# JJKK1313/DiTreeOnlinePlanner

Hardware: AMD Instinct MI355X
Metric: candidate tree-expansions/sec (carmaze, H=32) (higher is better)
Workload: dtype f16x3; 1 GPU; cfgs/carmaze.yaml + fm_policy flow sampler (K=1), batch=1024 candidates per GPU, H=32 (4 chunks x 8 steps), boxes.csv 20x20, 1024-node tree snapshot, seeded random weights; batch_per_gpu=1024, global_batch=1024, edge_length=32, action_horizon=8, pred_horizon=64, flow_steps=1, tree_nodes=1024, parallelism=candidates sharded x1

## Files before the change

ditreeonlineplanner_amd/csrc/conv_tiles.hip:

```cpp
#include <type_traits>

#include "denoise_device.h"

static thread_local bool g_dn_dry_run = false;
void denoise_set_dry_run(bool on) { g_dn_dry_run = on; }
bool denoise_dry_run() { return g_dn_dry_run; }

template <int PREC>
__device__ __forceinline__ void gemm_epilogue(const ConvGemmParams& p, f32x16_t (&acc)[2][4], char* smem, int tm, int tn,
                                              int tid, int lane, int r5, int h, int wm, int wn,
                                              long long out_extra_bytes = 0) {

  constexpr int ET = PREC == 2 ? 1 : 0;
  float satm = 0.0f;
  const int c_l = wn * 128 + 4 * r5;
  const int n0 = tn * 256 + c_l;
  const bool n_ok = n0 < p.N;
  float bias4[4] = {0.f, 0.f, 0.f, 0.f};
  if (p.bias != nullptr && n_ok) {
    f32x4_t t = *(const f32x4_t*)(p.bias + n0);
#pragma unroll
    for (int j = 0; j < 4; ++j) bias4[j] = t[j];
  }
#pragma unroll
// ... 1185 lines not shown
#pragma unroll
  for (int q = 0; q < 4; ++q) issue_w(v_lo, 1, q);
  rdA(0, v_lo, 0, 0);
  rdB(0, v_lo, 0, 1, 0);
#ifdef HALO16_STAMP
  const unsigned long long xs1 = __builtin_amdgcn_s_memrealtime();
#endif

  using IT1 = std::integral_constant<int, NP == 6 ? 3 : 2>;
  for (int v = v_lo; v < nv - 2; ++v) {
    step(I0{}, Tt{}, Tt{}, Tt{}, I3{}, v);
    step(I1{}, Tt{}, Tt{}, Tt{}, IT1{}, v);
    step(I2{}, Tt{}, Tt{}, Tt{}, I0{}, v);
  }
#ifdef X3_PHASE_STAMP
  if (blockIdx.x == 100 && lane == 0 && nv == 64) {
#pragma unroll
    for (int k = 0; k < 24; ++k) g_x3_phase[w][k] = pst[k];
    g_x3_phase[w][24] = (unsigned)nv;
  }
#endif
  {
    const int v = nv - 2;
    step(I0{}, Tt{}, Tt{}, Tt{}, I0{}, v);
    step(I1{}, Tt{}, Tt{}, Tt{}, I0{}, v);
    step(I2{}, Tt{}, Tt{}, Ff{}, I0{}, v);
  }
  {
    const int v = nv - 1;
    step(I0{}, Tt{}, Tt{}, Ff{}, I0{}, v);
    step(I1{}, Tt{}, Ff{}, Ff{}, I0{}, v);
    step(I2{}, Ff{}, Ff{}, Ff{}, I0{}, v);
  }
  __builtin_amdgcn_s_setprio(0);
  __syncthreads();
#ifdef HALO16_STAMP
  const unsigned long long xs2 = __builtin_amdgcn_s_memrealtime();
#endif
  if constexpr (SPLITK) {
    const int ntiles = ntm * ntn;
    float* mine = p.sk_ws + ((size_t)blockIdx.y * ntiles + tile) * 65536;
#pragma unroll
    for (int mb = 0; mb < 4; ++mb)
#pragma unroll
      for (int j = 0; j < 8; ++j) *(f32x4_t*)(mine + ((mb * 8 + j) * 512 + tid) * 4) = acc[mb][j];
    __threadfence();
    __syncthreads();
    int* s_last = (int*)smem;
    if (tid == 0) *s_last = atomicAdd(p.sk_cnt + tile, 1) == p.splitk - 1;
    __syncthreads();
    const bool last = *s_last != 0;
    __syncthreads();
    if (!last) return;
    __threadfence();
#pragma unroll
    for (int mb = 0; mb < 4; ++mb)
#pragma unroll
      for (int j = 0; j < 8; ++j) acc[mb][j] = f32x4_t{0.f, 0.f, 0.f, 0.f};
    for (int sp = 0; sp < p.splitk; ++sp) {
      const float* sl = p.sk_ws + ((size_t)sp * ntiles + tile) * 65536;
#pragma unroll
      for (int mb = 0; mb < 4; ++mb)
#pragma unroll
        for (int j = 0; j < 8; ++j) acc[mb][j] += *(const f32x4_t*)(sl + ((mb * 8 + j) * 512 + tid) * 4);
    }
    if (tid == 0) p.sk_cnt[tile] = 0;
  }
  gemm_epilogue16<ET, true, SHORT>(p, acc, smem, tm, tn, tid, lane, r4, h4, wm, wn);
#ifdef HALO16_STAMP
  __syncthreads();
  if (tid == 0) {
    const unsigned long long xs3 = __builtin_amdgcn_s_memrealtime();
    const unsigned int k = atomicAdd(&g_x3_count, 1u);
    if (k < X3_STAMP_MAX) {
      g_x3_stamp[k][0] = xs0; g_x3_stamp[k][1] = xs1; g_x3_stamp[k][2] = xs2; g_x3_stamp[k][3] = xs3;
      g_x3_stamp[k][4] = ((unsigned long long)nv << 32) | blockIdx.x;
      g_x3_stamp[k][5] = ((unsigned long long)__builtin_amdgcn_s_getreg((31 << 11) | 20) << 32) |
                         (unsigned int)__builtin_amdgcn_s_getreg((31 << 11) | 4);
    }
  }
#endif
}

template <int ET, bool SPLIT>
__global__ void __launch_bounds__(256) conv2d_small_kernel(ConvGemmParams p) {
  extern __shared__ __attribute__((aligned(16))) char smem[];
  constexpr int STAGE = 16384;
  constexpr int CK = SPLIT ? 32 : 64;
  const int tid = threadIdx.x, lane = tid & 63;
  const int w = __builtin_amdgcn_readfirstlane(tid >> 6);
  const int r5 = lane & 31, h = lane >> 5;
  const int wm = w >> 1, wn = w & 1;
  const int ntn = p.N >> 6;
  const int tm = blockIdx.x / ntn, tn = blockIdx.x - tm * ntn;
  const int kpt = p.Cin / CK;
  const long long K = (long long)p.taps * p.Cin;
  int k0 = 0, nk = p.taps * kpt;
  long long out_extra = 0;
  if (p.splitk > 1) {
    const int per = (nk + p.splitk - 1) / p.splitk;
    k0 = blockIdx.y * per;
    nk = min(nk - k0, per);
    out_extra = (long long)blockIdx.y * p.slab_stride;
  }

  const char* a_base[2];
  int ih0[2], iw0[2];
  const char* w_src[2];
  int slot_b[2];
  long long plane_a[2];
#pragma unroll
  for (int q = 0; q < 2; ++q) {
    const int r = (2 * w + q) * 8 + (lane >> 3);
    const int slot = (lane & 7) ^ ((r >> 1) & 7);
    slot_b[q] = SPLIT ? (slot & 3) * 16 : slot * 16;
    plane_a[q] = (SPLIT && (slot & 4)) ? p.a_plane : 0;
    const long long plane_w = (SPLIT && (slot & 4)) ? p.w_plane : 0;
    int m = tm * 64 + r;
    m = m < p.M ? m : p.M - 1;
    const int b = m / p.c2_OHW, rem = m - b * p.c2_OHW;
    const int oh = rem / p.c2_OW, ow = rem - oh * p.c2_OW;
    a_base[q] = (const char*)p.A + (long long)b * p.c2_H * p.c2_W * p.Cin * 2;
    ih0[q] = oh * p.c2_stride - p.c2_pad;
    iw0[q] = ow * p.c2_stride - p.c2_pad;
    w_src[q] = (const char*)p.W + ((long long)(tn * 64 + r) * K) * 2 + slot_b[q] + plane_w;
  }
  auto issue = [&](int kl) {
    const int k = k0 + kl;
    const int tap = k / kpt, kin = k - tap * kpt;
    const int kh = p.c2_kh[tap], kw = p.c2_kw[tap];
    char* st = smem + (kl % 3) * STAGE;
#pragma unroll
    for (int q = 0; q < 2; ++q) {
      const int ih = ih0[q] + kh, iw = iw0[q] + kw;
      const bool ok = ih >= 0 && ih < p.c2_H && iw >= 0 && iw < p.c2_W;
      const char* src = ok ? a_base[q] + ((long long)(ih * p.c2_W + iw) * p.Cin + kin * CK) * 2 + plane_a[q] : (const char*)p.zero;
      __builtin_amdgcn_global_load_lds((const GLOBAL_AS void*)(src + slot_b[q]), (LDS_AS void*)(st + (2 * w + q) * 1024), 16, 0, 0);
    }
#pragma unroll
    for (int q = 0; q < 2; ++q)
      __builtin_amdgcn_global_load_lds((const GLOBAL_AS void*)(w_src[q] + (long long)k * (CK * 2)),
                                       (LDS_AS void*)(st + 8192 + (2 * w + q) * 1024), 16, 0, 0);
  };

  f32x16_t acc;
#pragma unroll
  for (int i = 0; i < 16; ++i) acc[i] = 0.0f;
  const int a_row = wm * 32 + r5, b_row = wn * 32 + r5;
  const int a_off = a_row * 128, b_off = 8192 + b_row * 128;
  const int sa = (a_row >> 1) & 7, sb = (b_row >> 1) & 7;

  issue(0);
  if (nk > 1) issue(1);
  for (int k = 0; k < nk; ++k) {
    if (k + 1 < nk) asm volatile("s_waitcnt vmcnt(4)" ::: "memory");
    else asm volatile("s_waitcnt vmcnt(0)" ::: "memory");
    __builtin_amdgcn_s_barrier();
    if (k + 2 < nk) issue(k + 2);
    const char* st = smem + (k % 3) * STAGE;
    if constexpr (SPLIT) {
      short8_t af[4], bf[4];
#pragma unroll
      for (int ks = 0; ks < 4; ++ks) {
        af[ks] = *(const short8_t*)(st + a_off + ((((ks << 1) | h) ^ sa) << 4));
        bf[ks] = *(const short8_t*)(st + b_off + ((((ks << 1) | h) ^ sb) << 4));
      }
#pragma unroll
      for (int kk = 0; kk < 2; ++kk) acc = mfma32<ET>(af[kk], bf[kk + 2], acc);
#pragma unroll
      for (int kk = 0; kk < 2; ++kk) acc = mfma32<ET>(af[kk], bf[kk], acc);
#pragma unroll
      for (int kk = 0; kk < 2; ++kk) acc = mfma32<ET>(af[kk + 2], bf[kk], acc);
    } else {
#pragma unroll
      for (int ks = 0; ks < 4; ++ks) {
        const short8_t af = *(const short8_t*)(st + a_off + ((((ks << 1) | h) ^ sa) << 4));
        const short8_t bf = *(const short8_t*)(st + b_off + ((((ks << 1) | h) ^ sb) << 4));
        acc = mfma32<ET>(af, bf, acc);
      }
    }
    asm volatile("s_waitcnt lgkmcnt(0)" ::: "memory");
  }

  const int n = tn * 64 + wn * 32 + r5;
  float bias = (p.bias != nullptr && k0 == 0) ? p.bias[n] : 0.0f;
#pragma unroll
  for (int i = 0; i < 16; ++i) {
    const int m = tm * 64 + wm * 32 + (i & 3) + 8 * (i >> 2) + 4 * h;
    if (m < p.M) ((float*)p.Out)[out_extra + (long long)m * p.ldc + p.out_coff + n] = (ET == 1 ? acc[i] * p.w_scale : acc[i]) + bias;
  }
}

template <int ET, bool SPLIT, bool SHORT = false>
__global__ void __launch_bounds__(512, 2) gemm16_kernel(ConvGemmParams p) {
  extern __shared__ __attribute__((aligned(16))) char smem[];
  constexpr int BUF = 32768, W_BASE = 2 * BUF;
  const int tid = threadIdx.x, lane = tid & 63;
  const int w = __builtin_amdgcn_readfirstlane(tid >> 6);
  const int r4 = lane & 15, h4 = lane >> 4;
  const int wm = w >> 1, wn = w & 1;
  const int ntn = p.N >> 8, ntm = p.M >> 8;
  const int tile = xcd_remap_strips(blockIdx.x, ntm, ntn, p.xcd_strips);
  const int tm = tile / ntn, tn = tile - tm * ntn;
  constexpr int KB = SPLIT ? 64 : 128;
  const int nc = SPLIT ? (p.Cin >> 5) : (p.Cin >> 6), nk = p.taps * nc;
  const unsigned a_plane = (unsigned)p.a_plane, w_plane = (unsigned)p.w_plane;
  const long long K = (long long)p.taps * p.Cin;

  long long a_tile0;
  {
    const int m0 = tm * 256;
    const int b0 = m0 / p.L, l0 = m0 - b0 * p.L;
    a_tile0 = (((long long)b0 * p.in_Lp + (long long)l0 * p.in_stride + p.in_off) * p.lda) * 2;
  }
  const __amdgpu_buffer_rsrc_t a_rsrc =
      __builtin_amdgcn_make_buffer_rsrc((void*)((const char*)p.A + a_tile0), 0, 0x7fffffff, 0x00020000);
  const __amdgpu_buffer_rsrc_t w_rsrc =
      __builtin_amdgcn_make_buffer_rsrc((void*)((const char*)p.W + ((long long)tn * 256) * K * 2), 0, 0x7fffffff, 0x00020000);
  unsigned pae, pao, pbe, pbo;
  int aq[4], wq[4];
  {
    const int lr = lane >> 3;
    const int slot0 = (lane & 7) ^ (lr >> 1), slot1 = slot0 ^ 4;
    const int lrb = lr / p.L, lro = lrb * p.in_Lp + (lr - lrb * p.L) * p.in_stride;
    if constexpr (SPLIT) {
      pae = (unsigned)((lro * p.lda + (slot0 & 3) * 8) * 2) + ((slot0 & 4) ? a_plane : 0u);
      pao = (unsigned)((lro * p.lda + (slot1 & 3) * 8) * 2) + ((slot1 & 4) ? a_plane : 0u);
      pbe = (unsigned)(((long long)(8 * lr) * K + (slot0 & 3) * 8) * 2) + ((slot0 & 4) ? w_plane : 0u);
      pbo = (unsigned)(((long long)(8 * lr) * K + (slot1 & 3) * 8) * 2) + ((slot1 & 4) ? w_plane : 0u);
    } else {
      pae = (unsigned)((lro * p.lda + slot0 * 8) * 2);
      pao = (unsigned)((lro * p.lda + slot1 * 8) * 2);
      pbe = (unsigned)(((long long)(8 * lr) * K + slot0 * 8) * 2);
      pbo = (unsigned)(((long long)(8 * lr) * K + slot1 * 8) * 2);
    }
#pragma unroll
    for (int q = 0; q < 4; ++q) {
      const int r0 = (w * 4 + q) * 8;
      const int m = tm * 256 + r0;
      const int b = m / p.L, l = m - b * p.L;
      aq[q] = (int)((((long long)b * p.in_Lp + (long long)l * p.in_stride + p.in_off) * p.lda) * 2 - a_tile0);
      const int cu = (r0 & 128) + 8 * (r0 & 8) + ((r0 >> 4) & 7);
      wq[q] = (int)((long long)cu * K * 2);
    }
  }
  const int tap_bytes = p.lda * 2;
  auto src_off = [&](int k, int& ao, int& wo) {
    const int t = k / nc, c = k - t * nc;
    ao = t * tap_bytes + c * KB;
    wo = k * KB;
  };
  auto issue = [&](int kv) {
    int ao, wo;
    src_off(kv, ao, wo);
    char* ab = smem + (kv & 1) * BUF;
    char* wb = smem + W_BASE + (kv & 1) * BUF;
#pragma unroll
    for (int q = 0; q < 4; ++q)
      __builtin_amdgcn_raw_ptr_buffer_load_lds(a_rsrc, (LDS_AS void*)(ab + (w * 4 + q) * 1024), 16, (q & 1) ? pao : pae,
                                               aq[q] + ao, 0, 0);
#pragma unroll
    for (int q = 0; q < 4; ++q)
      __builtin_amdgcn_raw_ptr_buffer_load_lds(w_rsrc, (LDS_AS void*)(wb + (w * 4 + q) * 1024), 16, (q & 1) ? pbo : pbe,
                                               wq[q] + wo, 0, 0);
  };

// ... 78 lines not shown
      __builtin_amdgcn_sched_barrier(0);
      mm16(0, 1, 1);
      __builtin_amdgcn_sched_barrier(0);
    } else {
      rdB(1, k, 0, 1);
      mm16(0, 0, 0);
      __builtin_amdgcn_sched_group_barrier(0x100, 4, 0);
      __builtin_amdgcn_sched_group_barrier(0x008, 16, 0);
      __builtin_amdgcn_sched_barrier(0);
      rdA(1, k, 1);
      rdB(0, k, 1, 0);
      mm16(0, 1, 1);
      __builtin_amdgcn_sched_group_barrier(0x100, 8, 0);
      __builtin_amdgcn_sched_group_barrier(0x008, 16, 0);
      __builtin_amdgcn_sched_barrier(0);
      rdB(1, k, 1, 1);
      mm16(1, 0, 0);
      __builtin_amdgcn_sched_group_barrier(0x100, 4, 0);
      __builtin_amdgcn_sched_group_barrier(0x008, 16, 0);
      __builtin_amdgcn_sched_barrier(0);
    }
    int ao2 = 0, wo2 = 0;
    if constexpr (ISSUE) src_off(k + 2, ao2, wo2);
    if constexpr (HAS_NEXT) {
      asm volatile("s_waitcnt vmcnt(0) lgkmcnt(0)" ::: "memory");
      __builtin_amdgcn_s_barrier();
      rdA(0, k + 1, 0);
      rdB(0, k + 1, SPLIT ? 1 : 0, 0);
    }
#pragma unroll
    for (int mb = 0; mb < 4; ++mb)
#pragma unroll
      for (int jj = 0; jj < 4; ++jj) {
        mm(1, 1, 1, mb, (mb & 1) ? 3 - jj : jj);
        if constexpr (ISSUE) {
          const int m = mb * 4 + jj, i = (m & 1) ? -1 : (m >> 1);
          if (i >= 0 && i < 4)
            __builtin_amdgcn_raw_ptr_buffer_load_lds(a_rsrc, (LDS_AS void*)(smem + (k & 1) * BUF + (w * 4 + i) * 1024), 16,
                                                     (i & 1) ? pao : pae, aq[i] + ao2, 0, 0);
          else if (!SPLIT && i >= 4 && i < 8)
            __builtin_amdgcn_raw_ptr_buffer_load_lds(w_rsrc, (LDS_AS void*)(smem + W_BASE + (k & 1) * BUF + (w * 4 + i - 4) * 1024),
                                                     16, ((i - 4) & 1) ? pbo : pbe, wq[i - 4] + wo2, 0, 0);
        }
      }
    if constexpr (HAS_NEXT) __builtin_amdgcn_sched_group_barrier(0x100, 8, 1);
#pragma unroll
    for (int i = 0; i < 16; ++i) {
      __builtin_amdgcn_sched_group_barrier(0x008, 1, 1);
      if (ISSUE && !(i & 1) && (!SPLIT || i < 8)) __builtin_amdgcn_sched_group_barrier(0x020, 1, 1);
    }
    __builtin_amdgcn_sched_barrier(0);
  };
  using Tt = std::true_type;
  using Ff = std::false_type;

  issue(0);
  asm volatile("s_waitcnt vmcnt(0)" ::: "memory");
  __builtin_amdgcn_s_barrier();
  if (nk > 1) {
    if constexpr (SPLIT) {
      int ao, wo;
      src_off(1, ao, wo);
#pragma unroll
      for (int q = 0; q < 4; ++q)
        __builtin_amdgcn_raw_ptr_buffer_load_lds(a_rsrc, (LDS_AS void*)(smem + BUF + (w * 4 + q) * 1024), 16, (q & 1) ? pao : pae,
                                                 aq[q] + ao, 0, 0);
    } else {
      issue(1);
    }
  }
  rdA(0, 0, 0);
  rdB(0, 0, SPLIT ? 1 : 0, 0);
  for (int k = 0; k < nk - 2; ++k) step(Tt{}, Tt{}, k);
  if (nk >= 2) step(Tt{}, Ff{}, nk - 2);
  step(Ff{}, Ff{}, nk - 1);
  __syncthreads();
  gemm_epilogue16<ET, SPLIT, SHORT>(p, acc, smem, tm, tn, tid, lane, r4, h4, wm, wn);
}
enum { TILE_HALO, TILE_GEMM16, TILE_C2D_SMALL, TILE_GENERIC };
enum { TV_SPLIT = 1,
       TV_SHORT = 2,
       TV_SPLITK = 4,
       TV_NP6 = 8,
       TV_C2D = 16 };
struct TileVariant {
  void (*kernel)(ConvGemmParams);
  unsigned lds_bytes;
  unsigned block;
  int family, st;
  unsigned flags;
  int kind;
};
static const TileVariant k_tiles[] = {
    {conv3_halo16_kernel<0>, 147456, 512, TILE_HALO, ST_BF16, 0, 0},
    {conv3_halo16_kernel<1>, 147456, 512, TILE_HALO, ST_F16, 0, 0},
    {conv3_halo16x3_kernel<0>, 147456, 512, TILE_HALO, ST_BF16, TV_SPLIT, 0},
    {conv3_halo16x3_kernel<1>, 147456, 512, TILE_HALO, ST_F16, TV_SPLIT, 0},
    {conv3_halo16x3_kernel<0, true>, 147456, 512, TILE_HALO, ST_BF16, TV_SPLIT | TV_SHORT, 0},
    {conv3_halo16x3_kernel<1, true>, 147456, 512, TILE_HALO, ST_F16, TV_SPLIT | TV_SHORT, 0},
    {conv3_halo16x3_kernel<0, false, true>, 147456, 512, TILE_HALO, ST_BF16, TV_SPLIT | TV_SPLITK, 0},
    {conv3_halo16x3_kernel<1, false, true>, 147456, 512, TILE_HALO, ST_F16, TV_SPLIT | TV_SPLITK, 0},
    {conv3_halo16x3_kernel<0, true, true>, 147456, 512, TILE_HALO, ST_BF16, TV_SPLIT | TV_SHORT | TV_SPLITK, 0},
    {conv3_halo16x3_kernel<1, true, true>, 147456, 512, TILE_HALO, ST_F16, TV_SPLIT | TV_SHORT | TV_SPLITK, 0},
    {conv3_halo16x3_kernel<0, true, false, 6>, 163840, 512, TILE_HALO, ST_BF16, TV_SPLIT | TV_SHORT | TV_NP6, 0},
    {conv3_halo16x3_kernel<1, true, false, 6>, 163840, 512, TILE_HALO, ST_F16, TV_SPLIT | TV_SHORT | TV_NP6, 0},
    {gemm16_kernel<0, false>, 131072, 512, TILE_GEMM16, ST_BF16, 0, 1},
    {gemm16_kernel<1, false>, 131072, 512, TILE_GEMM16, ST_F16, 0, 1},
    {gemm16_kernel<0, true>, 131072, 512, TILE_GEMM16, ST_BF16, TV_SPLIT, 1},
    {gemm16_kernel<1, true>, 131072, 512, TILE_GEMM16, ST_F16, TV_SPLIT, 1},
    {gemm16_kernel<0, false, true>, 131072, 512, TILE_GEMM16, ST_BF16, TV_SHORT, 1},
    {gemm16_kernel<1, false, true>, 131072, 512, TILE_GEMM16, ST_F16, TV_SHORT, 1},
    {gemm16_kernel<0, true, true>, 131072, 512, TILE_GEMM16, ST_BF16, TV_SPLIT | TV_SHORT, 1},
    {gemm16_kernel<1, true, true>, 131072, 512, TILE_GEMM16, ST_F16, TV_SPLIT | TV_SHORT, 1},
    {conv2d_small_kernel<0, false>, 3 * 16384, 256, TILE_C2D_SMALL, ST_BF16, TV_C2D, 2},
    {conv2d_small_kernel<1, false>, 3 * 16384, 256, TILE_C2D_SMALL, ST_F16, TV_C2D, 2},
    {conv2d_small_kernel<0, true>, 3 * 16384, 256, TILE_C2D_SMALL, ST_BF16, TV_C2D | TV_SPLIT, 2},
    {conv2d_small_kernel<1, true>, 3 * 16384, 256, TILE_C2D_SMALL, ST_F16, TV_C2D | TV_SPLIT, 2},
    {conv_gemm_kernel<0, false>, 131072, 512, TILE_GENERIC, ST_BF16, 0, 1},
    {conv_gemm_kernel<1, false>, 131072, 512, TILE_GENERIC, ST_F32, 0, 1},
    {conv_gemm_kernel<2, false>, 131072, 512, TILE_GENERIC, ST_F16, 0, 1},
    {conv_gemm_kernel<0, true>, 131072, 512, TILE_GENERIC, ST_BF16, TV_C2D, 2},
    {conv_gemm_kernel<1, true>, 131072, 512, TILE_GENERIC, ST_F32, TV_C2D, 2},
    {conv_gemm_kernel<2, true>, 131072, 512, TILE_GENERIC, ST_F16, TV_C2D, 2},
};
static const TileVariant* find_tile(int family, int st, unsigned flags) {
  for (const TileVariant& v : k_tiles)
    if (v.family == family && v.st == st && v.flags == flags) return &v;
  return nullptr;
}

static const TileVariant* pick_tile(const ConvGemmParams& p, int fmt) {
  const int st = fmt_st(fmt);
  const bool split = fmt_split(fmt);
  const unsigned fsplit = split ? TV_SPLIT : 0;
  const bool tile16 = st != ST_F32 && !p.c2d && (p.M & 255) == 0 && (p.N & 255) == 0 && (p.Cin & 63) == 0;
  const bool l_ok = p.L >= 16 || (p.L == 8 && split) || (p.L == 4 && split && p.splitk <= 1);
  if (tile16 && p.taps == 3 && p.in_stride == 1 && p.in_Lp == p.L + 2 && (256 % p.L) == 0 && l_ok && p.Cin >= 192) {
    if (!split) return find_tile(TILE_HALO, st, 0);
    const unsigned fshort = p.L <= 8 ? TV_SHORT : 0;
    if (p.splitk > 1) return find_tile(TILE_HALO, st, TV_SPLIT | fshort | TV_SPLITK);
    return find_tile(TILE_HALO, st, TV_SPLIT | fshort | (p.L == 4 ? TV_NP6 : 0));
  }
  const bool short_l = p.L == 8 || p.L == 4;
  if (tile16 && (!p.out_f32 || p.mode == MODE_BIAS) && p.taps >= 1 && p.taps <= 3 && ((p.L & 15) == 0 || short_l) && p.M > 0 &&
      (p.mode == MODE_BIAS || (256 % p.L) == 0))
    return find_tile(TILE_GEMM16, st, fsplit | ((p.L & 15) != 0 ? TV_SHORT : 0));
  if (p.c2d && conv2d_small_eligible(fmt) && (p.N & 63) == 0 && (p.Cin & 63) == 0 && p.out_f32 && p.mode == MODE_BIAS)
    return find_tile(TILE_C2D_SMALL, st, TV_C2D | fsplit);
  if (split) return nullptr;
  return find_tile(TILE_GENERIC, st, p.c2d ? TV_C2D : 0);
}
bool conv2d_small_eligible(int fmt) { return fmt_st(fmt) != ST_F32; }
int conv_gemm_kind(const ConvGemmParams& p, int fmt) {
  const TileVariant* v = pick_tile(p, fmt);
  return v != nullptr ? v->kind : (p.c2d ? 2 : 1);
}
bool conv_gemm_supported(const ConvGemmParams& p, int fmt) { return pick_tile(p, fmt) != nullptr; }

static void ensure_lds_attrs() {
  static bool done[64] = {};
  int dev = 0;
  hipGetDevice(&dev);
  if (dev < 0 || dev >= 64 || done[dev]) return;
  done[dev] = true;
  for (const TileVariant& v : k_tiles)
    if (v.lds_bytes > 65536) hipFuncSetAttribute((const void*)v.kernel, hipFuncAttributeMaxDynamicSharedMemorySize, (int)v.lds_bytes);
}

void launch_conv_gemm(const ConvGemmParams& p, int fmt, hipStream_t s) {
  ensure_lds_attrs();
  const TileVariant* v = pick_tile(p, fmt);
  if (v != nullptr && (v->flags & TV_SPLITK) &&
      (p.sk_ws == nullptr || p.sk_cnt == nullptr || ((p.Cin >> 5) % p.splitk) != 0 || (p.Cin >> 5) / p.splitk < 2))
    throw std::runtime_error("conv_gemm: split-K of the halo kernel needs its workspace and splitk | Cin / 32, >= 2 chunks each");
  if ((v == nullptr || v->family == TILE_GENERIC) && p.mode >= MODE_GN_MISH && (p.L & 15) != 0)
    throw std::runtime_error("conv_gemm: a fused GroupNorm epilogue at L = 8 / 4 exists on the gemm16 tile only (whole 256-row tiles)");
  if (v == nullptr) throw std::runtime_error("conv_gemm: a split GEMM of this shape fits no tile (conv_gemm_supported is the contract)");
  dim3 grid(((p.M + 255) >> 8) * ((p.N + 255) >> 8));
  if (v->family == TILE_C2D_SMALL) grid.x = ((p.M + 63) >> 6) * (p.N >> 6);
  if (v->flags & (TV_SPLITK | TV_C2D)) grid.y = p.splitk > 1 ? p.splitk : 1;
  DN_LAUNCH(v->kernel, grid, dim3(v->block), v->lds_bytes, s, p);
}
```

ditreeonlineplanner_amd/csrc/denoise.h:

```cpp
#pragma once
#include <hip/hip_runtime.h>
#include <stdint.h>

enum { MODE_BIAS = 0, MODE_GN_MISH = 1, MODE_GN_MISH_FILM = 2, MODE_GN_MISH_RES = 3 };

enum { ST_BF16 = 0, ST_F32 = 1, ST_F16 = 2 };
static inline int fmt_make(int st, bool split) { return st | (split ? 4 : 0); }
static inline __host__ __device__ int fmt_st(int f) { return f & 3; }
static inline __host__ __device__ bool fmt_split(int f) { return (f & 4) != 0; }
static inline int fmt_es(int f) { return fmt_st(f) == ST_F32 ? 4 : 2; }

struct ConvGemmParams {
  const void* A;
  int lda;
  int in_Lp;
  int in_stride;
  int in_off;
  int taps, Cin;
  const void* W;
  void* Out;
  int ldc;
  int out_Lp, out_stride, out_off;
  int out_coff;
  int L;
  int M, N;
  const float* bias;
  int mode;
  const float* gamma;
  const float* beta;
  int group_ch;
  float eps;
  const float* film;
  int film_ld, film_off;
  const void* Res;
  int ldres, res_Lp, res_off;
  int out_f32;
  int xcd_strips;
  int c2d, c2_H, c2_W, c2_OW, c2_OHW, c2_stride, c2_pad;
  signed char c2_kh[12], c2_kw[12];
  const void* zero;
  long long a_plane, w_plane, out_plane, res_plane;
  float w_scale;
  int splitk;
  long long slab_stride;
  float* sk_ws;
  int* sk_cnt;
  int* sat;
};

void denoise_set_dry_run(bool on);
bool denoise_dry_run();
void launch_conv_gemm(const ConvGemmParams& p, int fmt, hipStream_t s);
bool conv2d_small_eligible(int fmt);
int conv_gemm_kind(const ConvGemmParams& p, int fmt);
bool conv_gemm_supported(const ConvGemmParams& p, int fmt);
void launch_prep_sample(const float* x, void* A0, int B, int P, int D, int fmt, long long plane, hipStream_t s, int* sat = nullptr);
void launch_time_embed(float t, const float* W1, const float* b1, const float* W2, const float* b2, float* out,
                       hipStream_t s);
void launch_prep_cond(const float* temb, const float* map_emb, int E, int E_ld, const float* cond, int G, void* out, int B,
                      int Kpad, int fmt, long long plane, hipStream_t s, int* sat = nullptr);
struct FlowStep {
  int mode;
  float dt;
  float sb, sa, c0, c1, sigma;
  const float* z;
  long long z_row;
  const int* z_idx;
  int z_row0;
};
void launch_final_proj_flow(const void* Y, int C, int Lp, long long plane, const float* W, const float* bias, int D, float* x,
                            FlowStep fs, const double* act_norm , double* actions, int B, int P, int fmt,
                            hipStream_t s);
struct TapList {
  int n;
  signed char kh[49], kw[49];
};
void launch_gn1d(void* x, int ld, int Lp, int row_off, int coff, int L, int C, const float* gamma, const float* beta, float eps,
                 int mode, const float* film, int film_ld, int film_off, const void* res, int ldres, int res_Lp, int res_off,
                 int B, int fmt, long long x_plane, long long res_plane, hipStream_t s, int* sat = nullptr);
void launch_encoder_stem(const float* lm, int n, const float* W, const float* gamma, const float* beta, void* out, int B, float eps,
                         int fmt, long long plane, hipStream_t s, int* sat = nullptr);
void launch_im2col2d(const void* in, bool src_f32, void* out, int B, int H, int W, int C, const TapList& taps, int stride,
                     int pad, int OH, int OW, int Kpad, int fmt, hipStream_t s);
void launch_gn2d(const float* in, int nslab, long long slab_stride, const float* gamma, const float* beta, const void* res,
                 int relu, void* out, int B, int HW, int C, float eps, int fmt, long long res_plane, long long out_plane,
                 hipStream_t s, int* sat = nullptr);
void launch_maxpool2d(const void* in, void* out, int B, int H, int W, int C, int OH, int OW, int fmt, hipStream_t s);
void launch_avgpool2d(const void* in, void* out, int B, int HW, int C, int fmt, long long in_plane, long long out_plane,
                      hipStream_t s);
void launch_unpack_act(const void* in, int ld, int coff, int Lp, int roff, float* out, int B, int L, int C, int fmt,
                       long long plane, hipStream_t s);

enum { ENC_RESNET = 0, ENC_IDENTITY = 1, ENC_MLP = 2, ENC_MAX = 3, ENC_GRID = 4, ENC_CNN = 5 };
struct SmallEncoderParams {
  int kind;
  const float* lm;
  float* out;
  int B, n, E, k;
  const float* w[4];
  const float* b[4];
};
const char* small_encoder_name(int kind);
int small_encoder_width(int kind, int n, int k);
void launch_small_encoder(const SmallEncoderParams& p, hipStream_t s);
```

ditreeonlineplanner_amd/csrc/denoise_host.hip:

```cpp
#include <algorithm>
#include <cmath>
#include <cstring>
#include <functional>
#include <map>
#include <sstream>
#include <thread>

#include "denoise.h"
#include "ditree_internal.h"

namespace {

struct HostParam {
  std::vector<int64_t> dims;
  const float* data = nullptr;
  int64_t n = 0;
};

struct Act {
  void* p = nullptr;
  int L = 0, C = 0;
  int ld = 0, coff = 0;
  bool padded = true;
  long long plane = 0;
// ... 599 lines not shown
    q.kind = enc_kind; q.n = lm; q.E = E; q.k = enc_k;
    auto transposed = [&](const std::string& name, int out_f, int in_f) {
      const HostParam& w = P_(name);
      if (w.dims.size() != 2 || w.dims[0] != out_f || w.dims[1] != in_f)
        throw std::runtime_error(name + " must be (" + std::to_string(out_f) + ", " + std::to_string(in_f) + ")");
      std::vector<float> t((size_t)out_f * in_f);
      for (int o = 0; o < out_f; ++o)
        for (int i = 0; i < in_f; ++i) t[(size_t)i * out_f + o] = w.data[(size_t)o * in_f + i];
      return upload_f32(name + "#t", t.data(), (int64_t)t.size());
    };
    auto conv_w = [&](const std::string& name, int co, int ci) {
      const HostParam& w = P_(name + ".weight");
      const HostParam& b = P_(name + ".bias");
      if (w.dims.size() != 4 || w.dims[0] != co || w.dims[1] != ci || w.dims[2] != 3 || w.dims[3] != 3 || b.n != co)
        throw std::runtime_error(name + " must be a Conv2d(" + std::to_string(ci) + ", " + std::to_string(co) + ", 3)");
    };
    if (enc_kind == ENC_MLP) {
      const int in_f = lm * lm;
      q.w[0] = transposed("encoder.fc1.weight", 128, in_f);
      q.w[1] = transposed("encoder.fc2.weight", 256, 128);
      q.w[2] = transposed("encoder.fc3.weight", E, 256);
      const int outs[3] = {128, 256, E};
      for (int l = 0; l < 3; ++l) {
        const std::string bn = "encoder.fc" + std::to_string(l + 1) + ".bias";
        if (P_(bn).n != outs[l]) throw std::runtime_error(bn + " must have " + std::to_string(outs[l]) + " elements");
        q.b[l] = vec(bn);
      }
    } else if (enc_kind == ENC_GRID || enc_kind == ENC_CNN) {
      const bool g = enc_kind == ENC_GRID;
      const int nl = g ? 3 : 4;
      const int ci[4] = {1, g ? 3 : 2, g ? 6 : 4, 4}, co[4] = {g ? 3 : 2, g ? 6 : 4, 4, 4};
      for (int l = 0; l < nl; ++l) {
        const std::string nm = "encoder.conv" + std::to_string(l + 1);
        conv_w(nm, co[l], ci[l]);
        q.w[l] = vec(nm + ".weight");
        q.b[l] = vec(nm + ".bias");
      }
    }
    const float** lm_slot = &lm_ptr;
    float* op = map_emb;
    const int LM = lm * lm, Ew = E;
    enc_ops.push_back([=, this](int b0, int Bn, int, hipStream_t s) {
      note_other();
      SmallEncoderParams r = q;
      r.lm = *lm_slot + (size_t)b0 * LM; r.out = op + (size_t)b0 * Ew; r.B = Bn;
      launch_small_encoder(r, s);
    });
  } else {
    const std::string R = "encoder.resnet18.";
    const int pr = efmt;
    const size_t E_ = ees();
    zero_row = dalloc(256);
    const size_t col_per_sample = 25 * 576;
    const size_t gout_per_sample = 9216;
    col_region = (size_t)sub_cap * col_per_sample;
    gout_region = (size_t)sub_cap * gout_per_sample;
    char* col = (char*)dalloc(col_region * ENC_SUBS * E_);
    float* gout = (float*)dalloc(gout_region * ENC_SUBS * 4);
    const size_t colreg = col_region, goutreg = gout_region;
    auto ebuf = [&](const std::string& name, int HW, int C) {
      Act a;
      a.L = HW; a.C = C; a.ld = C; a.coff = 0; a.padded = false; a.fmt = efmt;
      const size_t rows = HW == 1 ? (size_t)Brows : (size_t)Bmax;
      const size_t bytes = rows * HW * C * ees();
      a.plane = fmt_split(efmt) ? (long long)bytes : 0;
      a.p = dalloc(bytes * (fmt_split(efmt) ? 2 : 1));
      named[name] = a;
      return a;
    };
    auto live_taps = [](int k, int stride, int pad, int H, int OH) {
      TapList tl{};
      for (int kh = 0; kh < k; ++kh)
        for (int kw = 0; kw < k; ++kw) {
          bool lh = false, lw = false;
          for (int o = 0; o < OH; ++o) {
            const int ih = o * stride + kh - pad, iw = o * stride + kw - pad;
            lh |= (ih >= 0 && ih < H);
            lw |= (iw >= 0 && iw < H);
          }
          if (lh && lw) { tl.kh[tl.n] = (signed char)kh; tl.kw[tl.n] = (signed char)kw; ++tl.n; }
        }
      return tl;
    };
    auto conv2d = [&](const std::string& wname, const void* in, long long in_plane, int H, int Cin, int Cout, int k, int stride,
                      int pad, int OH, bool fold_in) {
      const HostParam& w = P_(wname + ".weight");
      const float* wd = w.data;
      const int Cw = (int)w.dims[1];
      const TapList tl = live_taps(k, stride, pad, H, OH);
      const int K = tl.n * Cin, Kpad = (K + 63) / 64 * 64;
      if ((size_t)OH * OH * Kpad > col_per_sample || (size_t)OH * OH * Cout > gout_per_sample)
        throw std::runtime_error("encoder scratch region too small for " + wname);
      const Packed wp = pack(wname, efmt, Cout, 1, Kpad, [=](int n, int, int kk) {
        if (kk >= K) return 0.0f;
        const int c = kk % Cin, t = kk / Cin, kw = tl.kw[t], kh = tl.kh[t];
        if (!fold_in) return wd[(((size_t)n * Cw + c) * k + kh) * k + kw];
        float s = 0.f;
        for (int cc = 0; cc < Cw; ++cc) s += wd[(((size_t)n * Cw + cc) * k + kh) * k + kw];
        return s;
      });
      const float** lm_slot = &lm_ptr;
      const bool implicit = (in != nullptr) && (Cin % 64 == 0) && tl.n <= 12;
      if (!implicit && fmt_split(efmt)) throw std::runtime_error("split encoder: " + wname + " needs the im2col path");
      const void* zr = zero_row;
      enc_ops.push_back([=, this](int b0, int Bn, int reg, hipStream_t s) {
        char* colr = col + (size_t)reg * colreg * E_;
        float* goutr = gout + (size_t)reg * goutreg;
        ConvGemmParams p{};
        const int M = Bn * OH * OH;
        if (implicit) {
          p.A = (const char*)in + (size_t)b0 * H * H * Cin * E_; p.lda = Cin; p.taps = tl.n; p.Cin = Cin; p.a_plane = in_plane;
          p.c2d = 1; p.c2_H = H; p.c2_W = H; p.c2_OW = OH; p.c2_OHW = OH * OH; p.c2_stride = stride; p.c2_pad = pad;
          for (int t = 0; t < tl.n; ++t) { p.c2_kh[t] = tl.kh[t]; p.c2_kw[t] = tl.kw[t]; }
          p.zero = zr;
          const int nk_total = tl.n * (Cin / 64);
          const int tiles = ((1024 * OH * OH + 255) / 256) * ((Cout + 255) / 256);
          static int sk_target = -1, sk_cap = 8;
          if (sk_target < 0) {
            const char* e = getenv("DITREE_SPLITK_TARGET");
            sk_target = (e && atoi(e) > 0) ? atoi(e) : 256;
            const char* c = getenv("DITREE_SPLITK_CAP");
            if (c && atoi(c) > 0) sk_cap = atoi(c);
          }
          int sk = std::max(1, std::min(std::min(sk_cap, nk_total / 2), std::max(1, sk_target / tiles)));
          while (sk > 1 && (size_t)sk * OH * OH * Cout > gout_per_sample) --sk;
          if (sk > 1) {
            const int per = (nk_total + sk - 1) / sk;
            sk = (nk_total + per - 1) / per;
          }
          static int use_split = -1;
          if (use_split < 0) { const char* e = getenv("DITREE_SPLITK"); use_split = (e && !atoi(e)) ? 0 : 1; }
          if (conv2d_small_eligible(pr)) {
            static int small_target = -1;
            if (small_target < 0) { const char* e = getenv("DITREE_C2D_TARGET"); small_target = (e && atoi(e) > 0) ? atoi(e) : 768; }
            const int tiles64 = ((1024 * OH * OH + 63) / 64) * (Cout / 64);
            sk = std::max(1, std::min(std::min(8, nk_total / 2), small_target / tiles64));
            while (sk > 1 && (size_t)sk * OH * OH * Cout > gout_per_sample) --sk;
            if (sk > 1) {
              const int per = (nk_total + sk - 1) / sk;
              sk = (nk_total + per - 1) / per;
            }
          }
          if (!use_split) sk = 1;
          p.splitk = sk;
          p.slab_stride = (long long)M * Cout;
          last_splitk[reg] = sk;
          last_slab[reg] = p.slab_stride;
        } else {
          last_splitk[reg] = 1;
          last_slab[reg] = 0;
        }
        if (!implicit) {
          note_other();
          if (in == nullptr)
            launch_im2col2d(*lm_slot + (size_t)b0 * H * H, true, colr, Bn, H, H, 1, tl, stride, pad, OH, OH, Kpad, pr, s);
          else
            launch_im2col2d((const char*)in + (size_t)b0 * H * H * Cin * E_, false, colr, Bn, H, H, Cin, tl, stride, pad,
                            OH, OH, Kpad, pr, s);
          p.A = colr; p.lda = Kpad; p.taps = 1; p.Cin = Kpad;
        }
        p.in_Lp = M; p.in_stride = 1; p.in_off = 0;
        set_w(p, wp);
        p.Out = goutr; p.ldc = Cout; p.out_Lp = M; p.out_stride = 1; p.out_off = 0;
        p.L = M; p.M = M; p.N = Cout; p.mode = MODE_BIAS; p.out_f32 = 1;
        run_gemm(p, pr, s);
      });
    };
    auto gn = [&](const std::string& gname, const Act& out, const Act* res, bool relu) {
      float* ga = vec(gname + ".weight");
      float* be = vec(gname + ".bias");
      const char* rp = res ? (const char*)res->p : nullptr;
      char* op = (char*)out.p;
      const int HW = out.L, C = out.C;
      const long long rpl = res ? res->plane : 0, opl = out.plane;
      {
        const int pp = (C >= 64 && C <= 1024 && (C & (C - 1)) == 0) ? 256 / (C >> 2) : 0;
        if (pp == 0 || (HW + pp - 1) / pp > 7)
          throw std::runtime_error("encoder GroupNorm: unsupported map (" + std::to_string(HW) + " pixels x " + std::to_string(C) + " channels)");
      }
      int* gsat = sat_slot(gname, efmt);
      enc_ops.push_back([=, this](int b0, int Bn, int reg, hipStream_t s) {
        note_other();
        const size_t off = (size_t)b0 * HW * C * E_;
        launch_gn2d(gout + (size_t)reg * goutreg, last_splitk[reg], last_slab[reg], ga, be, rp ? rp + off : nullptr,
                    relu ? 1 : 0, op + off, Bn, HW, C, 1e-5f, pr, rpl, opl, s, gsat);
      });
    };
    const int H0 = lm;
    auto osz = [](int h, int k, int s, int p) { return (h + 2 * p - k) / s + 1; };
    const int H1 = osz(H0, 7, 2, 3);
    const int H2 = osz(H1, 3, 2, 1);
    Act c1 = ebuf("enc.c1", H1 * H1, 64);
    Act pool = ebuf("enc.pool", H2 * H2, 64);
    if (H0 == 20 || H0 == 16) {
      const HostParam& w = P_(R + "conv1.weight");
      const int Cw = (int)w.dims[1];
      std::vector<float> wf(64 * 49);
      for (int n = 0; n < 64; ++n)
        for (int t = 0; t < 49; ++t) {
          float sacc = 0.f;
          for (int cc = 0; cc < Cw; ++cc) sacc += w.data[((size_t)n * Cw + cc) * 49 + t];
          wf[t * 64 + n] = sacc;
        }
      float* wdev = upload_f32(R + "conv1.weight#folded", wf.data(), 64 * 49);
      float* ga = vec(R + "bn1.weight");
      float* be = vec(R + "bn1.bias");
      char* op = (char*)pool.p;
      const float** lm_slot = &lm_ptr;
      const long long ppl = pool.plane;
      int* ssat = sat_slot(R + "conv1", efmt);
      enc_ops.push_back([=, this](int b0, int Bn, int, hipStream_t s) {
        note_other();
        launch_encoder_stem(*lm_slot + (size_t)b0 * H0 * H0, H0, wdev, ga, be, op + (size_t)b0 * H2 * H2 * 64 * E_, Bn, 1e-5f, pr, ppl, s, ssat);
      });
    } else {
    conv2d(R + "conv1", nullptr, 0, H0, 1, 64, 7, 2, 3, H1, true);
    gn(R + "bn1", c1, nullptr, true);
    {
      const char* ip = (const char*)c1.p; char* op = (char*)pool.p;
      const int a = H1, b2 = H2;
      enc_ops.push_back([=, this](int b0, int Bn, int, hipStream_t s) {
        note_other();
        launch_maxpool2d(ip + (size_t)b0 * a * a * 64 * E_, op + (size_t)b0 * b2 * b2 * 64 * E_, Bn, a, a, 64, b2, b2, pr, s);
      });
    }
    }
    Act cur = pool;
    int Hc = H2, Cc = 64;
    const int chans[4] = {64, 128, 256, 512};
    for (int li = 0; li < 4; ++li) {
      for (int bi = 0; bi < 2; ++bi) {
        const std::string pre = R + "layer" + std::to_string(li + 1) + "." + std::to_string(bi);
        const int Cout = chans[li];
        const int stride = (bi == 0 && li > 0) ? 2 : 1;
        const int Ho = osz(Hc, 3, stride, 1);
        const std::string tag = "enc.l" + std::to_string(li + 1) + "." + std::to_string(bi);
        Act t1 = ebuf(tag + ".t", Ho * Ho, Cout);
        conv2d(pre + ".conv1", cur.p, cur.plane, Hc, Cc, Cout, 3, stride, 1, Ho, false);
        gn(pre + ".bn1", t1, nullptr, true);
        Act idt = cur;
        if (has(pre + ".downsample.0.weight")) {
          Act ds = ebuf(tag + ".ds", Ho * Ho, Cout);
          conv2d(pre + ".downsample.0", cur.p, cur.plane, Hc, Cc, Cout, 1, stride, 0, Ho, false);
          gn(pre + ".downsample.1", ds, nullptr, false);
          idt = ds;
        }
        Act o = ebuf(tag + ".out", Ho * Ho, Cout);
        conv2d(pre + ".conv2", t1.p, t1.plane, Ho, Cout, Cout, 3, 1, 1, Ho, false);
        gn(pre + ".bn2", o, &idt, true);
        cur = o;
        Hc = Ho;
        Cc = Cout;
      }
    }
    Act pooled = ebuf("enc.avg", 1, Cc);
    {
      const char* ip = (const char*)cur.p; char* op = (char*)pooled.p;
      const int HW = Hc * Hc, C = Cc;
      const long long ipl = cur.plane, opl = pooled.plane;
      enc_ops.push_back([=, this](int b0, int Bn, int, hipStream_t s) {
        note_other();
        launch_avgpool2d(ip + (size_t)b0 * HW * C * E_, op + (size_t)b0 * C * E_, Bn, HW, C, pr, ipl, opl, s);
      });
    }
    {
      const HostParam& w = P_(R + "fc.weight");
      const float* wd = w.data;
      const int Kf = (int)w.dims[1], Nf = (int)w.dims[0];
      const Packed wp = pack(R + "fc", efmt, Nf, 1, Kf, [=](int n, int, int ci) { return wd[(size_t)n * Kf + ci]; });
      const bool esplit = fmt_split(efmt);
      const int eld = E_ld;
      float* bd;
      if (esplit) {
        std::vector<float> bpad(eld, 0.0f);
        std::memcpy(bpad.data(), P_(R + "fc.bias").data, (size_t)Nf * 4);
        bd = upload_f32(R + "fc.bias#padded", bpad.data(), eld);
      } else {
        bd = vec(R + "fc.bias");
      }
      const char* ip = (const char*)pooled.p;
      float* op = map_emb;
      const long long ppl = pooled.plane;
      enc_ops.push_back([=, this](int b0, int Bn, int, hipStream_t s) {
        ConvGemmParams p{};
        const int Mr = esplit ? (Bn + 255) / 256 * 256 : Bn;
        p.A = ip + (size_t)b0 * Kf * E_; p.lda = Kf; p.in_Lp = Mr; p.in_stride = 1; p.in_off = 0; p.taps = 1; p.Cin = Kf;
        set_w(p, wp); p.a_plane = ppl;
        p.Out = op + (size_t)b0 * eld; p.ldc = eld; p.out_Lp = Mr; p.out_stride = 1; p.out_off = 0;
        p.L = Mr; p.M = Mr; p.N = esplit ? eld : Nf; p.bias = bd; p.mode = MODE_BIAS; p.out_f32 = 1;
        run_gemm(p, pr, s);
      });
    }
  }
  if (hipDeviceSynchronize() != hipSuccess) throw std::runtime_error("sync after build failed");
  {
    float* lm_dev = (float*)dalloc((size_t)bgran * lm * lm * 4);
    lm_ptr = lm_dev;
    denoise_set_dry_run(true);
    try {
      for (auto& op : enc_ops) op(0, bgran, 0, nullptr);
      film_op(bgran, bgran, nullptr);
      for (auto& op : unet_ops) op(bgran, bgran, nullptr);
    } catch (...) {
      denoise_set_dry_run(false);
      lm_ptr = nullptr;
      throw;
    }
    denoise_set_dry_run(false);
    lm_ptr = nullptr;
  }
}

static int parse_manifest(DenoiserState* st, const char* manifest, int64_t n_floats) {
  std::istringstream in(manifest);
  std::string line;
  while (std::getline(in, line)) {
    if (line.empty()) continue;
    if (line.rfind("#config", 0) == 0) {
      std::istringstream cs(line.substr(7));
      std::string key;
      int val;
      while (cs >> key >> val) {
        if (key == "pred_horizon") st->P = val;
        else if (key == "local_map_size") st->lm = val;
      }
      continue;
    }
    if (line.rfind("#encoder", 0) == 0) {
      std::istringstream cs(line.substr(8));
      std::string kind;
      if (!(cs >> kind)) return -1;
      st->enc_kind = -1;
      for (int k = ENC_RESNET; k <= ENC_CNN; ++k)
        if (kind == small_encoder_name(k)) st->enc_kind = k;
      if (st->enc_kind < 0) return -3;
      int e;
      if (cs >> e) st->enc_E = e;
      continue;
    }
// ... 396 lines not shown
```

Measured before the change: 19440 candidate expansions/s.

## Fuse GroupNorm, residual and ReLU into small encoder Conv2d kernel

Adds a GN variant of the small conv2d implicit-GEMM kernel that packs each sample's output pixels into a power-of-two row slot. After the MMA loop it stages the tile in LDS and computes per-group mean and variance with lane shuffles. It then applies gamma, beta, the optional residual and ReLU, and writes 16-bit (optionally split) output directly. This removes the f32 intermediate write, the separate GroupNorm launch, and the avgpool when the spatial size is 1. The cost is padding waste in the row slots and no split-K, and shapes with long K and few tiles fall back to the unfused path.

```diff
diff --git a/ditreeonlineplanner_amd/csrc/conv_tiles.hip b/ditreeonlineplanner_amd/csrc/conv_tiles.hip
--- a/ditreeonlineplanner_amd/csrc/conv_tiles.hip
+++ b/ditreeonlineplanner_amd/csrc/conv_tiles.hip
@@ -1291,7 +1291,7 @@
 #endif
 }
 
-template <int ET, bool SPLIT>
+template <int ET, bool SPLIT, bool GN = false>
 __global__ void __launch_bounds__(256) conv2d_small_kernel(ConvGemmParams p) {
   extern __shared__ __attribute__((aligned(16))) char smem[];
   constexpr int STAGE = 16384;
@@ -1306,7 +1306,7 @@
   const long long K = (long long)p.taps * p.Cin;
   int k0 = 0, nk = p.taps * kpt;
   long long out_extra = 0;
-  if (p.splitk > 1) {
+  if (!GN && p.splitk > 1) {
     const int per = (nk + p.splitk - 1) / p.splitk;
     k0 = blockIdx.y * per;
     nk = min(nk - k0, per);
@@ -1325,19 +1325,45 @@
     slot_b[q] = SPLIT ? (slot & 3) * 16 : slot * 16;
     plane_a[q] = (SPLIT && (slot & 4)) ? p.a_plane : 0;
     const long long plane_w = (SPLIT && (slot & 4)) ? p.w_plane : 0;
-    int m = tm * 64 + r;
-    m = m < p.M ? m : p.M - 1;
-    const int b = m / p.c2_OHW, rem = m - b * p.c2_OHW;
+    int b, rem;
+    bool live = true;
+    if constexpr (GN) {
+      b = tm * (64 >> p.c2_psl) + (r >> p.c2_psl);
+      rem = r & ((1 << p.c2_psl) - 1);
+      live = rem < p.c2_OHW && b < p.c2_nb;
+      if (!live) { b = 0; rem = 0; }
+    } else {
+      int m = tm * 64 + r;
+      m = m < p.M ? m : p.M - 1;
+      b = m / p.c2_OHW;
+      rem = m - b * p.c2_OHW;
+    }
     const int oh = rem / p.c2_OW, ow = rem - oh * p.c2_OW;
     a_base[q] = (const char*)p.A + (long long)b * p.c2_H * p.c2_W * p.Cin * 2;
     ih0[q] = oh * p.c2_stride - p.c2_pad;
     iw0[q] = ow * p.c2_stride - p.c2_pad;
+    if constexpr (GN) { if (!live) ih0[q] = -(1 << 20); }
     w_src[q] = (const char*)p.W + ((long long)(tn * 64 + r) * K) * 2 + slot_b[q] + plane_w;
+  }
+  unsigned long long kh_tab = 0, kw_tab = 0;
+  if constexpr (GN) {
+#pragma unroll
+    for (int t = 0; t < 12; ++t) {
+      kh_tab |= (unsigned long long)(p.c2_kh[t] & 15) << (4 * t);
+      kw_tab |= (unsigned long long)(p.c2_kw[t] & 15) << (4 * t);
+    }
   }
   auto issue = [&](int kl) {
     const int k = k0 + kl;
     const int tap = k / kpt, kin = k - tap * kpt;
-    const int kh = p.c2_kh[tap], kw = p.c2_kw[tap];
+    int kh, kw;
+    if constexpr (GN) {
+      kh = (int)(kh_tab >> (4 * tap)) & 15;
+      kw = (int)(kw_tab >> (4 * tap)) & 15;
+    } else {
+      kh = p.c2_kh[tap];
+      kw = p.c2_kw[tap];
+    }
     char* st = smem + (kl % 3) * STAGE;
 #pragma unroll
     for (int q = 0; q < 2; ++q) {
@@ -1391,6 +1417,80 @@
     asm volatile("s_waitcnt lgkmcnt(0)" ::: "memory");
   }
 
+  if constexpr (GN) {
+    constexpr int TS = 68;
+    float* tile = (float*)smem;
+    __syncthreads();
+#pragma unroll
+    for (int i = 0; i < 16; ++i)
+      tile[(wm * 32 + (i & 3) + 8 * (i >> 2) + 4 * h) * TS + wn * 32 + r5] = ET == 1 ? acc[i] * p.w_scale : acc[i];
+    __syncthreads();
+    const int psl = p.c2_psl, ps = 1 << psl;
+    const int cell = tid >> psl, px = tid & (ps - 1);
+    const int sl = cell >> 2, g = cell & 3;
+    const int b = tm * (64 >> psl) + sl;
+    const bool live = px < p.c2_OHW && b < p.c2_nb;
+    f32x4_t v[4];
+#pragma unroll
+    for (int j = 0; j < 4; ++j) v[j] = *(const f32x4_t*)(tile + ((sl << psl) + px) * TS + g * 16 + 4 * j);
+    float s = 0.f;
+    if (live) {
+#pragma unroll
+      for (int j = 0; j < 4; ++j) s += (v[j][0] + v[j][1]) + (v[j][2] + v[j][3]);
+    }
+    for (int o = ps >> 1; o > 0; o >>= 1) s += __shfl_xor(s, o);
+    const float inv_n = 1.0f / (float)(p.c2_OHW * 16);
+    const float mean = s * inv_n;
+    float q2 = 0.f;
+    if (live) {
+#pragma unroll
+      for (int j = 0; j < 4; ++j)
+#pragma unroll
+        for (int e = 0; e < 4; ++e) { const float d = v[j][e] - mean; q2 = fmaf(d, d, q2); }
+    }
+    for (int o = ps >> 1; o > 0; o >>= 1) q2 += __shfl_xor(q2, o);
+    const float rstd = rsqrtf(q2 * inv_n + p.eps);
+    float satm = 0.0f;
+    if (live) {
+      const int n0 = tn * 64 + g * 16;
+      const long long idx = ((long long)b * p.c2_OHW + px) * p.ldc + p.out_coff + n0;
+      const long long ridx = ((long long)b * p.c2_OHW + px) * p.ldres + n0;
+#pragma unroll
+      for (int j = 0; j < 4; ++j) {
+        const f32x4_t ga = *(const f32x4_t*)(p.gamma + n0 + 4 * j), be = *(const f32x4_t*)(p.beta + n0 + 4 * j);
+        float y[4];
+#pragma unroll
+        for (int e = 0; e < 4; ++e) y[e] = (v[j][e] - mean) * rstd * ga[e] + be[e];
+        if (p.Res != nullptr) {
+          const short4_t rh = *(const short4_t*)((const unsigned short*)p.Res + ridx + 4 * j);
+#pragma unroll
+          for (int e = 0; e < 4; ++e) y[e] += e2f<ET>((unsigned short)rh[e]);
+          if constexpr (SPLIT) {
+            const short4_t rl = *(const short4_t*)((const unsigned short*)((const char*)p.Res + p.res_plane) + ridx + 4 * j);
+#pragma unroll
+            for (int e = 0; e < 4; ++e) y[e] += e2f<ET>((unsigned short)rl[e]);
+          }
+        }
+        if (p.relu) {
+#pragma unroll
+          for (int e = 0; e < 4; ++e) y[e] = y[e] > 0.f ? y[e] : 0.f;
+        }
+        if constexpr (ET == 1) { sat_see2(satm, y[0], y[1]); sat_see2(satm, y[2], y[3]); }
+        short4_t o;
+#pragma unroll
+        for (int e = 0; e < 4; ++e) o[e] = (short)f2e<ET>(y[e]);
+        *(short4_t*)((unsigned short*)p.Out + idx + 4 * j) = o;
+        if constexpr (SPLIT) {
+          short4_t o2;
+#pragma unroll
+          for (int e = 0; e < 4; ++e) o2[e] = (short)f2e<ET>(y[e] - e2f<ET>((unsigned short)o[e]));
+          *(short4_t*)((unsigned short*)((char*)p.Out + p.out_plane) + idx + 4 * j) = o2;
+        }
+      }
+    }
+    if constexpr (ET == 1) sat_flush(p.sat, satm);
+    return;
+  }
   const int n = tn * 64 + wn * 32 + r5;
   float bias = (p.bias != nullptr && k0 == 0) ? p.bias[n] : 0.0f;
 #pragma unroll
@@ -1635,7 +1735,8 @@
        TV_SHORT = 2,
        TV_SPLITK = 4,
        TV_NP6 = 8,
-       TV_C2D = 16 };
+       TV_C2D = 16,
+       TV_GN2D = 32 };
 struct TileVariant {
   void (*kernel)(ConvGemmParams);
   unsigned lds_bytes;
@@ -1669,6 +1770,10 @@
     {conv2d_small_kernel<1, false>, 3 * 16384, 256, TILE_C2D_SMALL, ST_F16, TV_C2D, 2},
     {conv2d_small_kernel<0, true>, 3 * 16384, 256, TILE_C2D_SMALL, ST_BF16, TV_C2D | TV_SPLIT, 2},
     {conv2d_small_kernel<1, true>, 3 * 16384, 256, TILE_C2D_SMALL, ST_F16, TV_C2D | TV_SPLIT, 2},
+    {conv2d_small_kernel<0, false, true>, 3 * 16384, 256, TILE_C2D_SMALL, ST_BF16, TV_C2D | TV_GN2D, 2},
+    {conv2d_small_kernel<1, false, true>, 3 * 16384, 256, TILE_C2D_SMALL, ST_F16, TV_C2D | TV_GN2D, 2},
+    {conv2d_small_kernel<0, true, true>, 3 * 16384, 256, TILE_C2D_SMALL, ST_BF16, TV_C2D | TV_SPLIT | TV_GN2D, 2},
+    {conv2d_small_kernel<1, true, true>, 3 * 16384, 256, TILE_C2D_SMALL, ST_F16, TV_C2D | TV_SPLIT | TV_GN2D, 2},
     {conv_gemm_kernel<0, false>, 131072, 512, TILE_GENERIC, ST_BF16, 0, 1},
     {conv_gemm_kernel<1, false>, 131072, 512, TILE_GENERIC, ST_F32, 0, 1},
     {conv_gemm_kernel<2, false>, 131072, 512, TILE_GENERIC, ST_F16, 0, 1},
@@ -1686,6 +1791,14 @@
   const int st = fmt_st(fmt);
   const bool split = fmt_split(fmt);
   const unsigned fsplit = split ? TV_SPLIT : 0;
+  if (p.mode == MODE_GN2D) {
+    const bool ok = p.c2d && st != ST_F32 && (p.N & 63) == 0 && (p.Cin & 63) == 0 && !p.out_f32 && p.splitk <= 1 && p.bias == nullptr &&
+                    p.gamma != nullptr && p.beta != nullptr && p.group_ch == 16 && p.c2_psl >= 0 && p.c2_psl <= 6 &&
+                    p.c2_OHW <= (1 << p.c2_psl) && p.c2_nb > 0 && p.M == p.c2_nb * p.c2_OHW && p.taps >= 1 && p.taps <= 12;
+    for (int t = 0; ok && t < p.taps; ++t)
+      if (p.c2_kh[t] < 0 || p.c2_kh[t] > 15 || p.c2_kw[t] < 0 || p.c2_kw[t] > 15) return nullptr;
+    return ok ? find_tile(TILE_C2D_SMALL, st, TV_C2D | fsplit | TV_GN2D) : nullptr;
+  }
   const bool tile16 = st != ST_F32 && !p.c2d && (p.M & 255) == 0 && (p.N & 255) == 0 && (p.Cin & 63) == 0;
   const bool l_ok = p.L >= 16 || (p.L == 8 && split) || (p.L == 4 && split && p.splitk <= 1);
   if (tile16 && p.taps == 3 && p.in_stride == 1 && p.in_Lp == p.L + 2 && (256 % p.L) == 0 && l_ok && p.Cin >= 192) {
@@ -1726,11 +1839,14 @@
   if (v != nullptr && (v->flags & TV_SPLITK) &&
       (p.sk_ws == nullptr || p.sk_cnt == nullptr || ((p.Cin >> 5) % p.splitk) != 0 || (p.Cin >> 5) / p.splitk < 2))
     throw std::runtime_error("conv_gemm: split-K of the halo kernel needs its workspace and splitk | Cin / 32, >= 2 chunks each");
+  if (v == nullptr && p.mode == MODE_GN2D)
+    throw std::runtime_error("conv_gemm: Conv2d + GroupNorm in one launch needs a 16-bit format, <= 64 pixels per sample and groups of 16");
   if ((v == nullptr || v->family == TILE_GENERIC) && p.mode >= MODE_GN_MISH && (p.L & 15) != 0)
     throw std::runtime_error("conv_gemm: a fused GroupNorm epilogue at L = 8 / 4 exists on the gemm16 tile only (whole 256-row tiles)");
   if (v == nullptr) throw std::runtime_error("conv_gemm: a split GEMM of this shape fits no tile (conv_gemm_supported is the contract)");
   dim3 grid(((p.M + 255) >> 8) * ((p.N + 255) >> 8));
   if (v->family == TILE_C2D_SMALL) grid.x = ((p.M + 63) >> 6) * (p.N >> 6);
+  if (v->flags & TV_GN2D) grid.x = ((p.c2_nb + (64 >> p.c2_psl) - 1) / (64 >> p.c2_psl)) * (p.N >> 6);
   if (v->flags & (TV_SPLITK | TV_C2D)) grid.y = p.splitk > 1 ? p.splitk : 1;
   DN_LAUNCH(v->kernel, grid, dim3(v->block), v->lds_bytes, s, p);
 }
diff --git a/ditreeonlineplanner_amd/csrc/denoise.h b/ditreeonlineplanner_amd/csrc/denoise.h
--- a/ditreeonlineplanner_amd/csrc/denoise.h
+++ b/ditreeonlineplanner_amd/csrc/denoise.h
@@ -2,7 +2,8 @@
 #include <hip/hip_runtime.h>
 #include <stdint.h>
 
-enum { MODE_BIAS = 0, MODE_GN_MISH = 1, MODE_GN_MISH_FILM = 2, MODE_GN_MISH_RES = 3 };
+enum { MODE_BIAS = 0, MODE_GN_MISH = 1, MODE_GN_MISH_FILM = 2, MODE_GN_MISH_RES = 3,
+       MODE_GN2D = 4 };
 
 enum { ST_BF16 = 0, ST_F32 = 1, ST_F16 = 2 };
 static inline int fmt_make(int st, bool split) { return st | (split ? 4 : 0); }
@@ -46,6 +47,8 @@
   float* sk_ws;
   int* sk_cnt;
   int* sat;
+  int c2_psl, c2_nb;
+  int relu;
 };
 
 void denoise_set_dry_run(bool on);
diff --git a/ditreeonlineplanner_amd/csrc/denoise_host.hip b/ditreeonlineplanner_amd/csrc/denoise_host.hip
--- a/ditreeonlineplanner_amd/csrc/denoise_host.hip
+++ b/ditreeonlineplanner_amd/csrc/denoise_host.hip
@@ -705,8 +705,9 @@
         }
       return tl;
     };
+    struct GnFuse { float* ga; float* be; int* sat; Act out; const char* res; long long res_plane; bool relu; };
     auto conv2d = [&](const std::string& wname, const void* in, long long in_plane, int H, int Cin, int Cout, int k, int stride,
-                      int pad, int OH, bool fold_in) {
+                      int pad, int OH, bool fold_in, const GnFuse* fz = nullptr) {
       const HostParam& w = P_(wname + ".weight");
       const float* wd = w.data;
       const int Cw = (int)w.dims[1];
@@ -726,6 +727,30 @@
       const bool implicit = (in != nullptr) && (Cin % 64 == 0) && tl.n <= 12;
       if (!implicit && fmt_split(efmt)) throw std::runtime_error("split encoder: " + wname + " needs the im2col path");
       const void* zr = zero_row;
+      if (fz != nullptr) {
+        if (!implicit) throw std::runtime_error("encoder: " + wname + " cannot take its GroupNorm into the conv launch");
+        const GnFuse f = *fz;
+        int psl = 0;
+        while ((1 << psl) < OH * OH) ++psl;
+        enc_ops.push_back([=, this](int b0, int Bn, int, hipStream_t s) {
+          ConvGemmParams p{};
+          const int M = Bn * OH * OH;
+          p.A = (const char*)in + (size_t)b0 * H * H * Cin * E_; p.lda = Cin; p.taps = tl.n; p.Cin = Cin; p.a_plane = in_plane;
+          p.c2d = 1; p.c2_H = H; p.c2_W = H; p.c2_OW = OH; p.c2_OHW = OH * OH; p.c2_stride = stride; p.c2_pad = pad;
+          for (int t = 0; t < tl.n; ++t) { p.c2_kh[t] = tl.kh[t]; p.c2_kw[t] = tl.kw[t]; }
+          p.zero = zr;
+          p.c2_psl = psl; p.c2_nb = Bn; p.relu = f.relu ? 1 : 0;
+          p.in_Lp = M; p.in_stride = 1; p.in_off = 0;
+          set_w(p, wp);
+          const size_t off = (size_t)b0 * OH * OH * Cout * E_;
+          p.Out = (char*)f.out.p + off; p.ldc = Cout; p.out_Lp = M; p.out_stride = 1; p.out_off = 0; p.out_plane = f.out.plane;
+          p.Res = f.res ? f.res + off : nullptr; p.ldres = Cout; p.res_plane = f.res_plane;
+          p.gamma = f.ga; p.beta = f.be; p.group_ch = 16; p.eps = 1e-5f; p.sat = f.sat;
+          p.L = M; p.M = M; p.N = Cout; p.mode = MODE_GN2D; p.out_f32 = 0; p.splitk = 1;
+          run_gemm(p, pr, s);
+        });
+        return;
+      }
       enc_ops.push_back([=, this](int b0, int Bn, int reg, hipStream_t s) {
         char* colr = col + (size_t)reg * colreg * E_;
         float* goutr = gout + (size_t)reg * goutreg;
@@ -809,6 +834,22 @@
                     relu ? 1 : 0, op + off, Bn, HW, C, 1e-5f, pr, rpl, opl, s, gsat);
       });
     };
+    auto conv_gn = [&](const std::string& wname, const std::string& gname, const Act& in, int H, int Cin, int Cout, int k, int stride,
+                       int pad, int OH, const Act& out, const Act* res, bool relu) {
+      const int ntaps = live_taps(k, stride, pad, H, OH).n;
+      int psl = 0;
+      while ((1 << psl) < OH * OH) ++psl;
+      const bool long_k_few_tiles = psl <= 6 && ntaps * Cin >= 2048 && (1024 >> (6 - psl)) * (Cout / 64) <= 256;
+      const bool fuse = conv2d_small_eligible(pr) && Cin % 64 == 0 && Cout % 64 == 0 && OH * OH <= 64 && ntaps <= 12 && !long_k_few_tiles;
+      if (!fuse) {
+        conv2d(wname, in.p, in.plane, H, Cin, Cout, k, stride, pad, OH, false);
+        gn(gname, out, res, relu);
+        return;
+      }
+      const GnFuse f{vec(gname + ".weight"), vec(gname + ".bias"), sat_slot(gname, efmt), out, res ? (const char*)res->p : nullptr,
+                     res ? res->plane : 0, relu};
+      conv2d(wname, in.p, in.plane, H, Cin, Cout, k, stride, pad, OH, false, &f);
+    };
     const int H0 = lm;
     auto osz = [](int h, int k, int s, int p) { return (h + 2 * p - k) / s + 1; };
     const int H1 = osz(H0, 7, 2, 3);
@@ -859,25 +900,22 @@
         const int Ho = osz(Hc, 3, stride, 1);
         const std::string tag = "enc.l" + std::to_string(li + 1) + "." + std::to_string(bi);
         Act t1 = ebuf(tag + ".t", Ho * Ho, Cout);
-        conv2d(pre + ".conv1", cur.p, cur.plane, Hc, Cc, Cout, 3, stride, 1, Ho, false);
-        gn(pre + ".bn1", t1, nullptr, true);
+        conv_gn(pre + ".conv1", pre + ".bn1", cur, Hc, Cc, Cout, 3, stride, 1, Ho, t1, nullptr, true);
         Act idt = cur;
         if (has(pre + ".downsample.0.weight")) {
           Act ds = ebuf(tag + ".ds", Ho * Ho, Cout);
-          conv2d(pre + ".downsample.0", cur.p, cur.plane, Hc, Cc, Cout, 1, stride, 0, Ho, false);
-          gn(pre + ".downsample.1", ds, nullptr, false);
+          conv_gn(pre + ".downsample.0", pre + ".downsample.1", cur, Hc, Cc, Cout, 1, stride, 0, Ho, ds, nullptr, false);
           idt = ds;
         }
         Act o = ebuf(tag + ".out", Ho * Ho, Cout);
-        conv2d(pre + ".conv2", t1.p, t1.plane, Ho, Cout, Cout, 3, 1, 1, Ho, false);
-        gn(pre + ".bn2", o, &idt, true);
+        conv_gn(pre + ".conv2", pre + ".bn2", t1, Ho, Cout, Cout, 3, 1, 1, Ho, o, &idt, true);
         cur = o;
         Hc = Ho;
         Cc = Cout;
       }
     }
-    Act pooled = ebuf("enc.avg", 1, Cc);
-    {
+    Act pooled = Hc == 1 ? cur : ebuf("enc.avg", 1, Cc);
+    if (Hc > 1) {
       const char* ip = (const char*)cur.p; char* op = (char*)pooled.p;
       const int HW = Hc * Hc, C = Cc;
       const long long ipl = cur.plane, opl = pooled.plane;
```

Measured after the change: 19600 candidate expansions/s (median of 6 runs). About the same (+0.8%).
